# lhaippp/DMHomo

Hardware: AMD Instinct MI355X
Metric: sampled images/sec (128x128, s_step=32) (higher is better)
Workload: dtype f32; 1 GPU; DGM CFG-Unet dim=64 128x128 bs=25/GPU s_step=32 cond_scale=3 (BASELINE configs[1]); global_batch=25, cfg_mode=streams, hip_graph=True, weights=seeded random init

## Files before the change

dmhomo_amd/_lib.py:

```python
import contextlib
import ctypes as C
import gc
import os

import torch

_HERE = os.path.dirname(os.path.abspath(__file__))
LIB_PATH = os.environ.get('DMH_LIB_PATH') or os.path.join(_HERE, 'libdmhomo_hip.so')

c_f32p = C.c_void_p
c_i64 = C.c_int64
c_int = C.c_int
c_float = C.c_float


ABI_VERSION = 500


class DmhConv(C.Structure):
    _fields_ = [('struct_size', C.c_uint64)] + \
               [(n, C.c_void_p) for n in ('src0', 'src1', 'wpack', 'bias', 'in_coef', 'res', 'res_coef', 'out',
                                          'stats')] + \
               [(n, C.c_int32) for n in ('B', 'Hin', 'Win', 'C0', 'C1', 'Cout', 'KH', 'KW', 'stride', 'upsample2')] + \
               [('in_bound', C.c_void_p), ('in_bound_n', C.c_int32), ('fin_n', C.c_int32), ('fin_w', C.c_void_p),
                ('fin_b', C.c_void_p), ('fin_out', C.c_void_p), ('pix_stats', C.c_void_p), ('pix_eps', C.c_float),
                ('rows', C.c_void_p)]


class DmhPackJob(C.Structure):
    _fields_ = [('src', C.c_void_p), ('ws', C.c_void_p), ('wpack', C.c_void_p), ('Cout', C.c_int32), ('C0', C.c_int32),
                ('C1', C.c_int32), ('KH', C.c_int32), ('transposed', C.c_int32)]


class DmhStep(C.Structure):
    _fields_ = [('objective', C.c_int32), ('clip', C.c_int32), ('mode', C.c_int32), ('cond_scale', C.c_float),
                ('sqrt_recip_ac', C.c_float), ('sqrt_recipm1_ac', C.c_float), ('sqrt_ac', C.c_float),
                ('sqrt_1m_ac', C.c_float), ('c0', C.c_float), ('c1', C.c_float), ('c2', C.c_float)]


SIGNATURES = {
    'dmh_last_error': (C.c_char_p, []),
    'dmh_version': (c_int, []),
    'dmh_ws_standardize': (c_int, [c_f32p, c_f32p, c_int, c_int, c_float, C.c_void_p]),
    'dmh_conv_pack_floats': (c_i64, [c_int, c_int, c_int, c_int, c_int]),
    'dmh_pack_conv_weight': (c_int, [c_f32p, c_f32p, c_int, c_int, c_int, c_int, c_int, C.c_void_p]),
    'dmh_pack_conv_weights_multi': (c_int, [C.c_void_p, c_int, c_float, C.c_void_p]),
    'dmh_conv_up2_pack_floats': (c_i64, [c_int, c_int]),
    'dmh_pack_conv_weight_up2': (c_int, [c_f32p, c_f32p, c_int, c_int, C.c_void_p]),
    'dmh_conv_tiles': (c_int, [c_int, c_int, c_int, c_int]),
# ... 226 lines not shown
```

dmhomo_amd/csrc/common.h:

```cpp
#pragma once
#include <initializer_list>
#include <hip/hip_runtime.h>
#include <stdint.h>
#include <stdio.h>

#include "../../include/dmhomo_hip.h"

void dmh_set_error(const char* fmt, ...);

#define DMH_REQUIRE(cond, ...)   \
  do {                           \
    if (!(cond)) {               \
      dmh_set_error(__VA_ARGS__); \
      return DMH_EINVAL;         \
    }                            \
  } while (0)

#define DMH_CHECK_LAUNCH(name)                                        \
  do {                                                                \
    hipError_t e_ = hipGetLastError();                                \
    if (e_ != hipSuccess) {                                           \
      dmh_set_error("%s: launch failed: %s", name, hipGetErrorString(e_)); \
      return DMH_ELAUNCH;                                             \
    }                                                                 \
// ... 3 lines not shown
  do {                                                                                                            \
    static bool raised_ = false;                                                                                  \
    if (!raised_) {                                                                                               \
      hipError_t e_ = hipFuncSetAttribute(reinterpret_cast<const void*>(kern),                                    \
                                          hipFuncAttributeMaxDynamicSharedMemorySize, (int)(bytes));              \
      DMH_REQUIRE(e_ == hipSuccess, "%s: cannot raise the LDS limit to %d bytes: %s", name, (int)(bytes),         \
                  hipGetErrorString(e_));                                                                         \
      raised_ = true;                                                                                             \
    }                                                                                                             \
  } while (0)

static inline bool dmh_dims_ok(std::initializer_list<long long> dims, long long lo = 1, long long hi = 1 << 20) {
  for (long long d : dims)
    if (d < lo || d > hi) return false;
  return true;
}

static inline int cdiv(int a, int b) { return (a + b - 1) / b; }
static inline int64_t cdiv64(int64_t a, int64_t b) { return (a + b - 1) / b; }

__device__ __forceinline__ float silu_f(float x) { return x / (1.0f + expf(-x)); }

__device__ __forceinline__ float silu_fast(float x) { return x * __builtin_amdgcn_rcpf(1.0f + __expf(-x)); }

__device__ __forceinline__ float4 ld4(const float* p) { return *reinterpret_cast<const float4*>(p); }
__device__ __forceinline__ void st4(float* p, float4 v) { *reinterpret_cast<float4*>(p) = v; }

template <int CTRL>
__device__ __forceinline__ unsigned dmh_dpp(unsigned v) {
  return (unsigned)__builtin_amdgcn_update_dpp(0, (int)v, CTRL, 0xf, 0xf, false);
}
__device__ __forceinline__ unsigned dmh_xor16(unsigned v, unsigned* other) {
  const auto r = __builtin_amdgcn_permlane16_swap(v, v, false, false);
  *other = r[1];
  return r[0];
}
__device__ __forceinline__ unsigned dmh_xor32(unsigned v, unsigned* other) {
  const auto r = __builtin_amdgcn_permlane32_swap(v, v, false, false);
  *other = r[1];
  return r[0];
}
__device__ __forceinline__ float row16_sum(float v) {
  v += __uint_as_float(dmh_dpp<0xB1>(__float_as_uint(v)));
  v += __uint_as_float(dmh_dpp<0x4E>(__float_as_uint(v)));
  v += __uint_as_float(dmh_dpp<0x141>(__float_as_uint(v)));
  v += __uint_as_float(dmh_dpp<0x140>(__float_as_uint(v)));
// ... 76 lines not shown
```

dmhomo_amd/csrc/conv.hip:

```cpp
#include <stdlib.h>

#include "common.h"

#include "conv_args.h"
#include "weight_image.h"

template <int KH, int KW, int S, int UPS, int KC, int TH, int TW>
struct ConvCfg {
  static constexpr int BM = TH * TW;
  static constexpr int MB = BM / 128;
  static constexpr int IN_H = (TH - 1) * S + KH;
  static constexpr int IN_W = (TW - 1) * S + KW;
  static constexpr int IN_PIX = IN_H * IN_W;
  static constexpr int KCP = KC + 4;
  static constexpr int C4 = KC / 4;
  static constexpr int NLOAD = (IN_PIX * C4 + 255) / 256;
  static constexpr int WL = 64 * C4 / 256;
  static constexpr int PAD = (S == 1) ? (KH / 2) : (KH == 4 ? 1 : 0);
  static constexpr int IN_FLOATS = IN_PIX * KCP;
  static constexpr int W_FLOATS = 64 * KCP;
  static constexpr int EPI_BYTES = 4 * 32 * 68 * 4;
  static constexpr int MAIN_BYTES = (IN_FLOATS + 2 * W_FLOATS) * 4;
  static constexpr int LDS_BYTES = MAIN_BYTES > EPI_BYTES ? MAIN_BYTES : EPI_BYTES;
};
// ... 327 lines not shown
              "dmh_conv2d: input channels must be a multiple of 4 (got %d, %d)", d->C0, d->C1);
  DMH_REQUIRE(!(d->in_coef && d->src1), "dmh_conv2d: the GroupNorm prologue applies to a single source");
  DMH_REQUIRE(!(d->res_coef && !d->res), "dmh_conv2d: res_coef without res");
  DMH_REQUIRE(d->Cout % 4 == 0, "dmh_conv2d: Cout must be a multiple of 4 (got %d)", d->Cout);
  DMH_REQUIRE(!d->in_bound || (d->in_coef && d->in_bound_n > 0 && d->in_bound_n <= 64),
              "dmh_conv2d: in_bound needs in_coef and 1..64 bounds per sample (got %d)", d->in_bound_n);
  hipStream_t st = (hipStream_t)stream;
  const int Hout = conv_out_dim(d->Hin, d->KH, d->stride, d->upsample2);
  const int Wout = conv_out_dim(d->Win, d->KW, d->stride, d->upsample2);
  const int key = d->KH * 100 + d->stride * 10 + d->upsample2;
  DMH_REQUIRE(d->KH == d->KW, "dmh_conv2d: non-square kernel");
  if (d->fin_w) {
    DMH_REQUIRE(d->fin_out && d->fin_n > 0 && d->fin_n <= 8, "dmh_conv2d: fin_w needs fin_out and 1 <= fin_n <= 8 (got %d)",
                d->fin_n);
    DMH_REQUIRE(d->KH == 1 && d->stride == 1 && d->Cout <= 64 && use_f16x3(1, 1),
                "dmh_conv2d: the fused final projection rides on the 1x1 fp16-piece kernel with Cout <= 64 (got %dx%d, Cout %d)",
                d->KH, d->KW, d->Cout);
  } else {
    DMH_REQUIRE(d->out, "dmh_conv2d: null pointer");
  }
  DMH_REQUIRE(!d->pix_stats || (d->KH == 1 && d->stride == 1 && d->Cout == 64 && use_f16x3(1, 1)),
              "dmh_conv2d: pix_stats rides on the 1x1 fp16-piece kernel with Cout == 64 (got %dx%d, Cout %d)", d->KH, d->KW,
              d->Cout);
  switch (key) {
    case 110:
      if (use_f16x3(1, 1)) return dmh_f16x3_launch(d, Hout, Wout, st);
      return launch_conv<1, 1, 1, 0, 32, 16, 16>(d, Hout, Wout, st);
    case 310:
      switch (conv3_variant()) {
        case 6: return dmh_wino_launch(d, Hout, Wout, st);
        case 9: return dmh_f16x3_launch(d, Hout, Wout, st);
        default: return launch_conv<3, 3, 1, 0, 32, 16, 16, 2>(d, Hout, Wout, st);
      }
    case 311:
      switch (conv3_variant()) {
        case 6: return dmh_wino_launch(d, Hout, Wout, st);
        case 9: return dmh_f16x3_launch(d, Hout, Wout, st);
        default: return launch_conv<3, 3, 1, 1, 32, 16, 16, 2>(d, Hout, Wout, st);
      }
    case 312:
      DMH_REQUIRE(use_f16x3(3, 1) && !d->src1 && d->Cout % 64 == 0 && !d->stats,
                  "dmh_conv2d: the sub-pixel upsampling conv needs the fp16-piece kernels, one source, Cout %% 64 == 0, no stats");
      return dmh_f16x3_launch_up2(d, Hout, Wout, st);
    case 710:
      if (use_f16x3(7, 1)) return dmh_f16x3_launch(d, Hout, Wout, st);
      return launch_conv<7, 7, 1, 0, 16, 16, 16>(d, Hout, Wout, st);
// ... 15 lines not shown
```

dmhomo_amd/csrc/conv_args.h:

```cpp
#pragma once
#include "common.h"

typedef float floatx16 __attribute__((ext_vector_type(16)));

struct ConvArgs {
  const float* src0;
  const float* src1;
  const float* wpack;
  const float* bias;
  const float* in_coef;
  const float* res;
  const float* res_coef;
  float* out;
  float* stats;
  const float* oscale;
  const float* in_bound;
  int in_bound_n;
  int fin_n;
  const float* fin_w;
  const float* fin_b;
  float* fin_out;
  float* pix_stats;
  float pix_eps;
  int B, Hin, Win, C0, C1, Cout, Hout, Wout;
  int nch0, nch1, tilesX, tilesY;
  int ablate;
  int xcd;
  const int32_t* rows;
};


static inline ConvArgs fill_conv_args(const DmhConv* d, int Hout, int Wout, int KC, int TH, int TW) {
  ConvArgs a;
  a.src0 = d->src0;
  a.src1 = d->src1;
  a.wpack = d->wpack;
  a.bias = d->bias;
  a.in_coef = d->in_coef;
  a.res = d->res;
  a.res_coef = d->res_coef;
  a.out = d->out;
  a.stats = d->stats;
  a.oscale = nullptr;
  a.in_bound = d->in_coef ? d->in_bound : nullptr;
  a.in_bound_n = d->in_bound_n;
  a.fin_n = d->fin_w ? d->fin_n : 0;
  a.fin_w = d->fin_w;
  a.fin_b = d->fin_b;
  a.fin_out = d->fin_out;
  a.pix_stats = d->pix_stats;
  a.pix_eps = d->pix_eps;
  a.B = d->B;
  a.Hin = d->Hin;
  a.Win = d->Win;
  a.C0 = d->C0;
  a.C1 = d->src1 ? d->C1 : 0;
  a.Cout = d->Cout;
  a.Hout = Hout;
  a.Wout = Wout;
  a.nch0 = cdiv(a.C0, KC);
  a.nch1 = cdiv(a.C1, KC);
  a.tilesX = cdiv(Wout, TW);
  a.tilesY = cdiv(Hout, TH);
  a.ablate = 0;
  a.xcd = 1;
  a.rows = d->rows;
  return a;
}


int64_t dmh_wino_pack_floats(int Cout, int C0, int C1);
int dmh_wino_pack(const float* w, float* wpack, int Cout, int C0, int C1, hipStream_t st);
int dmh_wino_launch(const DmhConv* d, int Hout, int Wout, hipStream_t st);


int64_t dmh_f16x3_pack_floats(int Cout, int C0, int C1, int KH, int KW);
int dmh_f16x3_pack(const float* w, float* wpack, int Cout, int C0, int C1, int KH, int KW, hipStream_t st);
int dmh_f16x3_launch(const DmhConv* d, int Hout, int Wout, hipStream_t st);
int dmh_f16x3_pack_multi(const DmhPackJob* jobs, int njobs, float eps, hipStream_t st);
int64_t dmh_f16x3_up2_pack_floats(int Cout, int C0);
int dmh_f16x3_up2_pack(const float* w, float* wpack, int Cout, int C0, hipStream_t st);
int dmh_f16x3_launch_up2(const DmhConv* d, int Hout, int Wout, hipStream_t st);


struct EpilogueRows {
  static constexpr int EP = 68;
  int b, n0, chn, c4, rsub;
  bool cok;
  float4 bias, ra, rb, s1, s2, osc;
// ... 223 lines not shown
```

dmhomo_amd/csrc/conv_f16x3.hip:

```cpp
#include <stdlib.h>

#include "common.h"

#include "conv_args.h"
#include "weight_image.h"

typedef _Float16 half8 __attribute__((ext_vector_type(8)));
typedef _Float16 half4 __attribute__((ext_vector_type(4)));
typedef float float4v __attribute__((ext_vector_type(4)));

namespace {

constexpr int KC = 32;
constexpr int PITCH = 160;
constexpr int STEP_U4 = 4 * 64;

template <int KH, int KW, int S, int UPS, int TH, int TW, int WM, int WN>
struct F16Cfg {
  static_assert(WM * WN == 4, "four waves per workgroup");
  static constexpr bool SUB = UPS == 3;
  static_assert(SUB || TH * TW == WM * 64, "64 pixels per wave");
  static_assert(!SUB || (KH == 2 && KW == 2 && S == 1 && TH == 4 && TW == 16 && WM == 4 && WN == 1), "sub-pixel geometry");
  static constexpr int IN_H = SUB ? TH + 2 : (TH - 1) * S + KH;
  static constexpr int IN_W = SUB ? TW + 2 : (TW - 1) * S + KW;
  static constexpr int IN_PIX = IN_H * IN_W;
  static constexpr int QS = UPS == 4 ? 2 : 3, NQ = 1 << QS;
  static constexpr int NLOAD = (IN_PIX * NQ + 255) / 256;
  static constexpr int PAD = UPS == 2 ? 0 : ((S == 1) ? (KH / 2) : (KH == 4 ? 1 : 0));
  static constexpr int ROWP = IN_W * PITCH;
  static constexpr int IN_BYTES = IN_H * ROWP;
  static constexpr int EPI_BYTES = 4 * 32 * EpilogueRows::EP * 4;
  static constexpr int TILE_BYTES = IN_BYTES > EPI_BYTES ? IN_BYTES : EPI_BYTES;
  static constexpr int LDS_BYTES = TILE_BYTES + 16;
};

__device__ __forceinline__ unsigned absbits(float x) { return __float_as_uint(x) & 0x7fffffffu; }

__device__ __forceinline__ int64_t f16x3_frag_floats_dev(int Cout, int C0, int C1, int T) {
  return (int64_t)((Cout + 63) / 64) * ((C0 + KC - 1) / KC + (C1 + KC - 1) / KC) * T * 2 * STEP_U4 * 4;
}

}

template <int KH, int KW, int S, int UPS, int TH, int TW, int WM, int WN>
__global__ __launch_bounds__(256, 2) void conv_f16x3_kernel(ConvArgs p) {
  using Cfg = F16Cfg<KH, KW, S, UPS, TH, TW, WM, WN>;
  constexpr bool PK = UPS == 4;
  constexpr int IN_W = Cfg::IN_W, IN_PIX = Cfg::IN_PIX, NLOAD = Cfg::NLOAD, NTAPS = PK ? (KH * KW + 1) / 2 : KH * KW,
                ROWP = Cfg::ROWP;

  extern __shared__ __attribute__((aligned(16))) float lds[];
  unsigned char* in_tile = reinterpret_cast<unsigned char*>(lds);
  unsigned* mxslot = reinterpret_cast<unsigned*>(in_tile + Cfg::TILE_BYTES);

  const int tid = threadIdx.x;
  const int lane = tid & 63;
  const int wave = tid >> 6;
  const int wave_u = __builtin_amdgcn_readfirstlane(wave);
  const int kg = lane >> 4;
  const int l15 = lane & 15;
  const int wm = wave / WN, wn = wave % WN;

  int t = blockIdx.x, by = blockIdx.y, nb = gridDim.x;
  if (p.rows) {
    nb = p.tilesX * p.tilesY * p.rows[0];
    const int lin = t + by * (int)gridDim.x;
    if (lin >= nb * (int)gridDim.y) return;
    t = lin % nb;
    by = lin / nb;
  }
// ... 51 lines not shown
#pragma unroll
    for (int nb = 0; nb < 4; ++nb) acc[mb][nb] = float4v{0.f, 0.f, 0.f, 0.f};

  const int nchunks = p.nch0 + p.nch1;
  const int nsteps = nchunks * NTAPS * 2;
  const uint4* wbase = reinterpret_cast<const uint4*>(p.wpack) + (size_t)__builtin_amdgcn_readfirstlane(nt) * nsteps * STEP_U4;

  constexpr bool ROWREUSE = KH == 3 && KW == 3 && S == 1 && UPS != 3 && UPS != 2;
  constexpr int NSTEP = NTAPS * 2;
  constexpr int NB = (NSTEP % 3 == 0 && WN != 1) ? 3 : 2;
  uint4 bq[NB][4];
  auto tap_of = [](int pos) constexpr { return ROWREUSE ? (pos % 3) * 3 + pos / 3 : pos; };
  auto load_b = [&](int buf, int ch_, int st_) {
    if (st_ >= NSTEP) {
      st_ -= NSTEP;
      ch_ += 1;
    }
    if (ch_ >= nchunks) ch_ = nchunks - 1;
    const uint4* src = wbase + ((size_t)(ch_ * NTAPS + tap_of(st_ >> 1)) * 2 + (st_ & 1)) * STEP_U4;
#pragma unroll
    for (int i = 0; i < 4; ++i) bq[buf][i] = src[i * 64 + lane];
  };
#pragma unroll
  for (int i = 0; i < NB - 1; ++i) load_b(i, 0, i);

  constexpr int QS = Cfg::QS, NQ = Cfg::NQ;
  const int c4 = tid & (NQ - 1);
  float4 v[NLOAD];
  constexpr bool PACKPW = KH == 3 && KW == 3 && S == 1 && UPS == 0 && WN == 1;
  int poff[NLOAD], wroff[PACKPW ? 1 : NLOAD];
  const int y0c = min(max(iy0, 0), Hlim - 1), x0c = min(max(ix0, 0), Wlim - 1);
  const int pbase = PACKPW ? (b * p.Hin + y0c) * p.Win + x0c : 0;
  unsigned inside = 0;
#pragma unroll
  for (int i = 0; i < NLOAD; ++i) {
    const int pix = (tid + i * 256) >> QS;
    const int pixc = pix < IN_PIX ? pix : IN_PIX - 1;
    const int wro = (pixc / IN_W) * ROWP + (pixc % IN_W) * PITCH + c4 * 8;
    if (!PACKPW) wroff[i] = wro;
    const int yy = iy0 + pixc / IN_W, xx = ix0 + pixc % IN_W;
    const bool ok = pix < IN_PIX && yy >= 0 && yy < Hlim && xx >= 0 && xx < Wlim;
    const int yc = min(max(yy, 0), Hlim - 1), xc = min(max(xx, 0), Wlim - 1);
    const int sy = UPS == 1 ? (yc >> 1) : yc, sx = UPS == 1 ? (xc >> 1) : xc;
    poff[i] = UPS == 2 ? ((yc << 16) | xc) : (b * p.Hin + sy) * p.Win + sx;
    if (PACKPW) poff[i] = (int)((unsigned)wro | ((unsigned)((yc - y0c) * p.Win + (xc - x0c)) << 16));
    inside |= (ok ? 1u : 0u) << i;
  }
  unsigned inside_ch = inside;
  const float* ld_src = p.src0;
  int ld_C = p.C0, ld_c = 0, ld_py = 0, ld_px = 0;
  auto issue_prep = [&](int ch) {
    const bool s1 = ch >= p.nch0;
    ld_src = s1 ? p.src1 : p.src0;
    ld_C = s1 ? p.C1 : p.C0;
    if (UPS == 2) {
      const int nchc = p.C0 / KC, par = ch / nchc;
      ld_py = par >> 1;
      ld_px = par & 1;
      ld_c = (ch - par * nchc) * KC + c4 * 4;
      inside_ch = 0u;
    } else {
      const int c = (s1 ? ch - p.nch0 : ch) * KC + c4 * 4;
      ld_c = c < ld_C ? c : 0;
    }
  };
  auto issue_one = [&](int i) {
    const float* a;
    if (UPS == 2) {
      const int ry = 2 * (poff[i] >> 16) - 1 + ld_py, rx = 2 * (poff[i] & 0xffff) - 1 + ld_px;
      const bool ok = ((inside >> i) & 1u) && ry >= 0 && ry < p.Hin && rx >= 0 && rx < p.Win;
      const int yc = min(max(ry, 0), p.Hin - 1), xc = min(max(rx, 0), p.Win - 1);
      a = ld_src + ((size_t)(b * p.Hin + yc) * p.Win + xc) * ld_C + ld_c;
      inside_ch |= (ok ? 1u : 0u) << i;
    } else {
      if (PACKPW) a = ld_src + (size_t)pbase * ld_C + (int)(((unsigned)poff[i] >> 16) * (unsigned)ld_C + (unsigned)ld_c);
      else a = ld_src + (size_t)poff[i] * ld_C + ld_c;
    }
#ifdef DMH_STAMPS
    a = (p.ablate & 32) ? ld_src + ld_c : a;
#endif
    v[i] = ld4(a);
  };
  issue_prep(0);
#pragma unroll
  for (int i = 0; i < NLOAD; ++i) issue_one(i);
  __syncthreads();
#ifdef DMH_STAMPS
  if (p.ablate & 128) {
    const float* gs = p.src0 + (size_t)b * p.Hin * p.Win * p.C0;
    double q1 = 0.0, q2 = 0.0;
#pragma unroll
    for (int j = 0; j < 4; ++j) {
      const float2 t2 = *reinterpret_cast<const float2*>(gs + (size_t)(((tid & 31) + 32 * j) * 8 + (tid >> 5)) * 2);
      q1 += (double)t2.x;
      q2 += (double)t2.y;
    }
    for (int off = 16; off; off >>= 1) {
      q1 += __shfl_xor(q1, off);
      q2 += __shfl_xor(q2, off);
    }
    const double nn = (double)p.Hin * p.Win * (p.C0 / 8);
    const double mean = q1 / nn;
    double var = q2 / nn - mean * mean;
    var = var < 0.0 ? 0.0 : var;
// ... 35 lines not shown
  }
  for (int ch = 0; ch < nchunks; ++ch) {
    const bool s1c = ch >= p.nch0;
    const bool pro = (p.in_coef != nullptr) && !s1c;
    float4 ca = make_float4(1.f, 1.f, 1.f, 1.f), cb = make_float4(0.f, 0.f, 0.f, 0.f);
    if (pro) {
      const int cq = ch * KC + c4 * 4;
      const int ccq = cq < p.C0 ? cq : 0;
      ca = ld4(p.in_coef + (size_t)(b * 2 + 0) * p.C0 + ccq);
      cb = ld4(p.in_coef + (size_t)(b * 2 + 1) * p.C0 + ccq);
    }
    const bool cvalid = UPS == 2 || (s1c ? ch - p.nch0 : ch) * KC + c4 * 4 < (s1c ? p.C1 : p.C0);
    const unsigned msk = cvalid ? inside_ch : 0u;
    if (pro) {
#pragma unroll
      for (int i = 0; i < NLOAD; ++i) {
        if ((i + 1) * 256 > IN_PIX * NQ && ((wave_u * 64 + i * 256) >> QS) >= IN_PIX) continue;
        v[i].x = silu_fast(fmaf(ca.x, v[i].x, cb.x));
        v[i].y = silu_fast(fmaf(ca.y, v[i].y, cb.y));
        v[i].z = silu_fast(fmaf(ca.z, v[i].z, cb.z));
        v[i].w = silu_fast(fmaf(ca.w, v[i].w, cb.w));
      }
    }
    if (!stat) {
      float mxf = 0.f;
#pragma unroll
      for (int i = 0; i < NLOAD; ++i) {
        if (pro && (i + 1) * 256 > IN_PIX * NQ && ((wave_u * 64 + i * 256) >> QS) >= IN_PIX) continue;
        mxf = fmaxf(fmaxf(mxf, fmaxf(fabsf(v[i].x), fabsf(v[i].y))), fmaxf(fabsf(v[i].z), fabsf(v[i].w)));
      }
      unsigned mx = __float_as_uint(mxf);
      mx = wave_max_u32(mx);
      if (lane == 0) atomicMax(&mxslot[ch & 1], mx);
    }
    STAMP(0)
    __syncthreads();
    STAMP(1)
    const int e_old = e_run;
    int e_ch = e_fix;
    if (!stat) {
      const unsigned bmx = mxslot[ch & 1];
      if (tid == 0) mxslot[(ch + 1) & 1] = 0u;
      e_ch = min(max((int)(__builtin_amdgcn_readfirstlane(bmx) >> 23), 16), 254);
    }
    e_run = max(e_run, e_ch);
    const float sc = __uint_as_float((unsigned)(268 - e_run) << 23);
    if (e_run != e_old && ch > 0) {
      const int fe = 127 + e_old - e_run;
      const float f = fe > 0 ? __uint_as_float((unsigned)fe << 23) : 0.f;
#pragma unroll
      for (int mb = 0; mb < 4; ++mb)
#pragma unroll
        for (int nb = 0; nb < 4; ++nb) acc[mb][nb] *= f;
    }
    const bool more = ch + 1 < nchunks;
    if (more) issue_prep(ch + 1);
#ifdef DMH_STAMPS
    if (p.ablate & 1) {
#pragma unroll
      for (int i = 0; i < NLOAD; ++i)
        if (more) issue_one(i);
    } else
#endif
#pragma unroll
    for (int i = 0; i < NLOAD; ++i) {
      if ((i + 1) * 256 <= IN_PIX * NQ || ((tid + i * 256) >> QS) < IN_PIX) {
        const float si = ((msk >> i) & 1u) ? sc : 0.f;
        uint2 h1, h2;
        dmh_split2(v[i].x, v[i].y, si, h1.x, h2.x);
        dmh_split2(v[i].z, v[i].w, si, h1.y, h2.y);
        int slot = PACKPW ? poff[i] : wroff[i];
        if (PACKPW) asm volatile("v_and_b32 %0, 0xffff, %0" : "+v"(slot));
        unsigned char* dst = in_tile + slot;
        *reinterpret_cast<uint2*>(dst) = h1;
        *reinterpret_cast<uint2*>(dst + 64) = h2;
      }
      if (more) issue_one(i);
    }
    STAMP(2)
    __syncthreads();
    STAMP(3)
    __builtin_amdgcn_sched_barrier(0);

    half8 a[4][2];
    half8 ar[ROWREUSE ? 5 : 1][2];
    auto read_a = [&](int tap) {
      const unsigned char* at = in_tile + (tap / KW) * ROWP + (tap % KW) * PITCH;
      if constexpr (PK) {
        const int t0 = 2 * tap, t1 = 2 * tap + 1 < KH * KW ? 2 * tap + 1 : 2 * tap;
        const int o0 = (t0 / KW) * ROWP + (t0 % KW) * PITCH, o1 = (t1 / KW) * ROWP + (t1 % KW) * PITCH;
        at = in_tile + ((kg >> 1) ? o1 : o0);
      }
#pragma unroll
      for (int mb = 0; mb < 4; ++mb)
#pragma unroll
        for (int pl = 0; pl < 2; ++pl) a[mb][pl] = *reinterpret_cast<const half8*>(at + arow[mb] + pl * 64);
    };
    auto read_rows = [&](int kx, int r0, int r1) {
      const unsigned char* at = in_tile + kx * PITCH;
#pragma unroll
      for (int r = r0; r < r1; ++r)
#pragma unroll
        for (int pl = 0; pl < 2; ++pl)
          ar[ROWREUSE ? r % 5 : 0][pl] = *reinterpret_cast<const half8*>(at + arow[0] + r * ROWP + pl * 64);
    };
#ifdef DMH_STAMPS
    if (!(p.ablate & 2))
#endif
    {
#pragma unroll
      for (int st = 0; st < NSTEP; ++st) {
#ifdef DMH_STAMPS
        if (!(p.ablate & 8))
#endif
        load_b((st + NB - 1) % NB, ch, st + NB - 1);
        __builtin_amdgcn_sched_barrier(0);
        const int pos = st >> 1;
#ifdef DMH_STAMPS
        if (!(p.ablate & 16) || st == 0)
#endif
        {
          if (ROWREUSE) {
            if ((st & 1) == 0) read_rows(pos / 3, pos % 3 == 0 ? 0 : 3 + pos % 3, 4 + pos % 3);
          } else if ((st & 1) == 0) {
            read_a(pos);
          }
        }
        auto afrag = [&](int mb, int pl) -> half8 {
          if constexpr (ROWREUSE) return ar[(mb + pos % 3) % 5][pl];
          else return a[mb][pl];
        };
#define DMH_A(mb, pl) afrag(mb, pl)
#pragma unroll
        for (int mb = 0; mb < 4; ++mb)
#pragma unroll
          for (int nb = 0; nb < 2; ++nb) {
            float4v& c = acc[mb][(st & 1) * 2 + nb];
            const half8 g1 = __builtin_bit_cast(half8, bq[st % NB][nb * 2]), g2 = __builtin_bit_cast(half8, bq[st % NB][nb * 2 + 1]);
            const half8 h1 = DMH_A(mb, 0), h2 = DMH_A(mb, 1);
            asm("v_mfma_f32_16x16x32_f16 %0, %1, %4, %0\n\t"
                "v_mfma_f32_16x16x32_f16 %0, %2, %3, %0\n\t"
                "v_mfma_f32_16x16x32_f16 %0, %1, %3, %0"
                : "+v"(c) : "v"(g1), "v"(g2), "v"(h1), "v"(h2));
          }
#undef DMH_A
      }
    }
#pragma unroll
    for (int mb = 0; mb < 4; mb += 2)
      asm volatile("s_nop 15" : "+v"(acc[mb][0]), "+v"(acc[mb][1]), "+v"(acc[mb][2]), "+v"(acc[mb][3]), "+v"(acc[mb + 1][0]),
                   "+v"(acc[mb + 1][1]), "+v"(acc[mb + 1][2]), "+v"(acc[mb + 1][3]));
    __builtin_amdgcn_sched_barrier(0);
    STAMP(4)
  }

#ifdef DMH_STAMPS
  if (!(p.ablate & 4))
#endif
  {
    constexpr int EP = EpilogueRows::EP;
    const float inv_s = __uint_as_float((unsigned)(e_run - 14) << 23);
    float* wl = lds + wave * (32 * EP);
    EpilogueRows er(p, b, n0);
    if (UPS == 3 && p.oscale) er.osc = ld4(p.oscale + nt * 64 + er.c4 * 4);
    er.osc.x *= inv_s;
    er.osc.y *= inv_s;
    er.osc.z *= inv_s;
    er.osc.w *= inv_s;
    __syncthreads();
#pragma unroll
    for (int hb = 0; hb < 2; ++hb) {
#pragma unroll
      for (int m2 = 0; m2 < 2; ++m2)
#pragma unroll
        for (int nb = 0; nb < 4; ++nb)
// ... 236 lines not shown
  return DMH_OK;
}

int dmh_f16x3_launch(const DmhConv* d, int Hout, int Wout, hipStream_t st) {
  const bool wide = d->Cout % 128 == 0;
  if (d->KH == 4) {
    return wide ? launch_f16x3<2, 2, 1, 2, 8, 16, 2, 2>(d, Hout, Wout, st)
                : launch_f16x3<2, 2, 1, 2, 16, 16, 4, 1>(d, Hout, Wout, st);
  }
  if (d->KH == 7) {
    if (f16x3_pk(d->C0, d->src1 ? d->C1 : 0, 7)) return launch_f16x3<7, 7, 1, 4, 16, 16, 4, 1>(d, Hout, Wout, st);
    return launch_f16x3<7, 7, 1, 0, 16, 16, 4, 1>(d, Hout, Wout, st);
  }
  if (d->KH == 1) {
    return wide ? launch_f16x3<1, 1, 1, 0, 8, 16, 2, 2>(d, Hout, Wout, st)
                : launch_f16x3<1, 1, 1, 0, 16, 16, 4, 1>(d, Hout, Wout, st);
  }
  if (d->upsample2) {
    return wide ? launch_f16x3<3, 3, 1, 1, 8, 16, 2, 2>(d, Hout, Wout, st)
                : launch_f16x3<3, 3, 1, 1, 16, 16, 4, 1>(d, Hout, Wout, st);
  }
  if (wide) return launch_f16x3<3, 3, 1, 0, 8, 16, 2, 2>(d, Hout, Wout, st);
  DMH_REQUIRE(17 * (int64_t)d->Win + 17 < 65536, "dmh_conv2d: 3x3 with Cout %% 128 != 0 supports Win <= 3853 (got %d)", d->Win);
  return launch_f16x3<3, 3, 1, 0, 16, 16, 4, 1>(d, Hout, Wout, st);
}
```

dmhomo_amd/csrc/norm.hip:

```cpp
#include "common.h"

__global__ __launch_bounds__(256) void gn_finalize_kernel(const float* __restrict__ stats, int tiles,
                                                          const float* __restrict__ gamma,
                                                          const float* __restrict__ beta, const float* __restrict__ ss,
                                                          int64_t ss_stride, float* __restrict__ coef, int C, int groups,
                                                          int hw, float eps, float* __restrict__ mr,
                                                          float* __restrict__ bound, const int32_t* __restrict__ rows) {
  __shared__ double red[2][4];
  __shared__ float bred[4];
  const int jb = blockIdx.x / groups, g = blockIdx.x % groups;
  if (jb >= dmh_rows_n(rows, gridDim.x / groups)) return;
  const int b = dmh_rows_phys(rows, jb);
  const int bg = b * groups + g;
  const int cg = C / groups;
  const int lane = threadIdx.x;
  double s1 = 0.0, s2 = 0.0;
  const int total = tiles * cg;
  for (int i = lane; i < total; i += 256) {
    const int tile = i / cg, cc = i % cg;
    const float2 st = *reinterpret_cast<const float2*>(stats + ((size_t)(b * tiles + tile) * C + g * cg + cc) * 2);
    s1 += (double)st.x;
    s2 += (double)st.y;
  }
  for (int off = 32; off; off >>= 1) {
// ... 45 lines not shown
__global__ __launch_bounds__(256) void gn_silu_residual_kernel(const float* __restrict__ y,
                                                               const float* __restrict__ coef,
                                                               const float* __restrict__ res, float* __restrict__ out,
                                                               int64_t per_sample4, int C, int64_t total4_all,
                                                               float* __restrict__ pstats, float eps,
                                                               const int32_t* __restrict__ rows) {
  const int C4 = C >> 2;
  const int lane = threadIdx.x & 63;
  const int64_t total4 = rows ? per_sample4 * rows[0] : total4_all;
  for (int64_t i0 = (int64_t)blockIdx.x * 256 + threadIdx.x; i0 - lane < total4; i0 += (int64_t)gridDim.x * 256) {
    const bool ok = i0 < total4;
    if (LPP == 0 && !ok) break;
    const int64_t il = ok ? i0 : total4 - 1;
    const int jb = (int)(il / per_sample4);
    const int b = dmh_rows_phys(rows, jb);
    const int64_t i = il + (int64_t)(b - jb) * per_sample4;
    const int c = (int)(i % C4) * 4;
    const float4 a = ld4(coef + (size_t)(b * 2 + 0) * C + c);
    const float4 bb = ld4(coef + (size_t)(b * 2 + 1) * C + c);
    const float4 v = ld4(y + i * 4);
    float4 r = make_float4(0.f, 0.f, 0.f, 0.f);
    if (res) r = ld4(res + i * 4);
    float4 o;
    o.x = silu_fast(fmaf(a.x, v.x, bb.x)) + r.x;
    o.y = silu_fast(fmaf(a.y, v.y, bb.y)) + r.y;
    o.z = silu_fast(fmaf(a.z, v.z, bb.z)) + r.z;
    o.w = silu_fast(fmaf(a.w, v.w, bb.w)) + r.w;
    if (ok) st4(out + i * 4, o);
    if (LPP > 0) {
      float s = 0.f;
      s += (o.x + o.y) + (o.z + o.w);
      s = lanes_sum<(LPP > 0 ? LPP : 1)>(s);
      const float mean = s / (float)C;
      float qsum = 0.f;
      const float dx = o.x - mean, dy = o.y - mean, dz = o.z - mean, dw = o.w - mean;
      qsum += (dx * dx + dy * dy) + (dz * dz + dw * dw);
      qsum = lanes_sum<(LPP > 0 ? LPP : 1)>(qsum);
      if (ok && (threadIdx.x % (LPP > 0 ? LPP : 1)) == 0) {
        const int64_t pix = i / C4;
        pstats[pix * 2 + 0] = mean;
        pstats[pix * 2 + 1] = 1.0f / sqrtf(qsum / (float)C + eps);
      }
    }
  }
}

template <int LPP, int NV>
__global__ __launch_bounds__(256) void chan_layernorm_kernel(const float* __restrict__ x, const float* __restrict__ g,
                                                             const float* __restrict__ res, float* __restrict__ out,
                                                             int64_t npix_all, int C, float eps,
// ... 216 lines not shown
```

dmhomo_amd/engine.py:

```python
import torch

from . import ops
from .layout import ATTN_SCALE, HIDDEN, sinusoidal_freq, unet_layout

FUSED_FINAL = True


class _Res:
    __slots__ = ('conv1', 'g1', 'b1', 'conv2', 'g2', 'b2', 'res', 'ss_off', 'cout')


class _Attn:
    __slots__ = ('linear', 'ln_g', 'qkv', 'pla', 'plo', 'out', 'out_g')


class UnetEngine:
    def __init__(self, module, groups=8):
        self.module = module
        self.groups = groups
        self._sig = None
        self._rows = None
        self._pert_lo = None

    def _signature(self):
        return (getattr(self.module, '_dmh_epoch', 0),) + tuple((p.data_ptr(), p._version) for p in self.module.parameters())

    def ensure_prepared(self):
        sig = self._signature()
# ... 65 lines not shown

        self.blocks = []
        for n in L.nodes:
            k = n.keys
            if n.kind == 'res':
                b = res(n)
            elif n.kind in ('linattn', 'attn'):
                b = attn(n)
            elif n.kind == 'unshuffle':
                w22 = f32(k['w']).reshape(n.cout, n.c0, 2, 2).contiguous()
                b = ops.PackedConv(w22, f32(k['b']), n.c0, 0, stride=2, batch=pb)
            else:
                b = conv(k['w'], k['b'], n.c0, stride=2 if n.kind == 'down4' else 1, ups=1 if n.kind == 'up3' else 0)
            self.blocks.append((n, b))
        pb.run()
        nxt = [b for _, b in self.blocks[1:]] + [None]
        self._pixel_stats = [isinstance(a, _Attn) and a.pla is not None for a in nxt]
        self.final_w = f32('final_conv.weight').reshape(L.out_dim, -1).contiguous()
        self.final_b = f32('final_conv.bias')
        res_nodes = [n for n in L.nodes if n.kind == 'res']
        self.mlp_wt = torch.cat([f32(n.keys['mlp_w']).t() for n in res_nodes], dim=1).contiguous()
        self.mlp_b = torch.cat([f32(n.keys['mlp_b']) for n in res_nodes]).contiguous()

    def _res(self, r, x0, x1, ss_all, pixel_stats=False, pre=None, final=None, keep_out=True, fin_out=None):
        B, H, W, _ = x0.shape
        hw = H * W
        rows = self._rows
        y1, st1 = pre if pre is not None else ops.conv2d(r.conv1, x0, x1, want_stats=True, rows=rows)
        ss = ss_all[:, r.ss_off:r.ss_off + 2 * r.cout]
        coef1, bound1 = ops.gn_finalize(st1, r.g1, r.b1, hw, self.groups, ss, want_bound=True, rows=rows)
        y2, st2 = ops.conv2d(r.conv2, y1, in_coef=coef1, want_stats=True, in_bound=bound1, rows=rows)
        coef2 = ops.gn_finalize(st2, r.g2, r.b2, hw, self.groups, rows=rows)
        if final is not None:
            return ops.conv2d(r.res, x0, x1, res=y2, res_coef=coef2, final=final, keep_out=keep_out, fin_out=fin_out, rows=rows)
        if r.res is not None:
            if pixel_stats and r.cout == 64 and r.res.k == 1 and ops.f16x3_default():
                return ops.conv2d(r.res, x0, x1, res=y2, res_coef=coef2, pixel_stats=True, rows=rows)
            x = ops.conv2d(r.res, x0, x1, res=y2, res_coef=coef2, rows=rows)
            return (x, None) if pixel_stats else x
        assert x1 is None
        if pixel_stats:
            if r.cout in ops.PIXEL_STATS_FUSABLE:
                return ops.gn_silu_residual(y2, coef2, x0, pixel_stats=True, rows=rows)
            return ops.gn_silu_residual(y2, coef2, x0, rows=rows), None
        return ops.gn_silu_residual(y2, coef2, x0, rows=rows)

    def _attn(self, a, x, stats=None):
        rows = self._rows
        if a.plo is not None:
            return ops.linear_attention_fused(x, a.ln_g, a.pla, ATTN_SCALE, out=a.plo, stats=stats, rows=rows)
        if a.pla is not None:
            o = ops.linear_attention_fused(x, a.ln_g, a.pla, ATTN_SCALE, stats=stats, rows=rows)
            y = ops.conv2d(a.out, o, rows=rows)
            return ops.chan_layernorm(y, a.out_g, res=x, rows=rows)
        xn = ops.chan_layernorm(x, a.ln_g, rows=rows)
        qkv = ops.conv2d(a.qkv, xn, rows=rows)
        if a.linear:
            o = ops.linear_attention_core(qkv, ATTN_SCALE, rows=rows)
            y = ops.conv2d(a.out, o, rows=rows)
            return ops.chan_layernorm(y, a.out_g, res=x, rows=rows)
        o = ops.attention_core(qkv, ATTN_SCALE, rows=rows, pert_lo=self._pert_lo)
        return ops.conv2d(a.out, o, res=x, rows=rows)

    def embed(self, time, class_rows, reps):
        B = time.shape[0]
        td = self.t_w2.shape[1]
        cond = torch.empty((reps * B, self.emb_dim), device=time.device, dtype=torch.float32)
        se = ops.fourier_embed(time, self.fourier_w) if self.fourier_w is not None else ops.sinusoidal_embed(time, self.freq)
# ... 31 lines not shown
    def first_conv(self, x0):
        self.ensure_prepared()
        return ops.conv2d(self.blocks[0][1].conv1, x0, None, want_stats=True)

    def trunk(self, x0, cond, taps=None, first=None, out=None, ss_all=None, rows=None, pert_lo=None):
        self.ensure_prepared()
        self._rows, self._pert_lo = rows, pert_lo
        try:
            return self._trunk(x0, cond, taps, first, out, ss_all)
        finally:
            self._rows = self._pert_lo = None

    def _trunk(self, x0, cond, taps, first, out, ss_all):
        rows = self._rows

        def tap(name, v):
            if taps is not None:
                taps[name] = v
            return v
        if ss_all is None:
            ss_all = ops.linear(cond, self.mlp_wt, self.mlp_b, act_in='silu')
        x = tap('init_conv', x0)
        hs, pst, last = [x], None, len(self.blocks) - 1
        for i, (n, b) in enumerate(self.blocks):
            x1 = hs.pop() if n.c1 else None
            if n.kind == 'res':
                if i == last and FUSED_FINAL and b.res is not None and b.res.k == 1 and b.cout <= 64 \
                        and self.final_w.shape[0] <= 8 and ops.f16x3_default():
                    x, y = self._res(b, x, x1, ss_all, final=(self.final_w, self.final_b), keep_out=taps is not None,
                                     fin_out=out)
                    tap(n.name, x)
                    return y
                if self._pixel_stats[i]:
                    x, pst = self._res(b, x, x1, ss_all, pixel_stats=True)
                else:
                    x = self._res(b, x, x1, ss_all, pre=first if i == 0 else None)
            elif n.kind in ('linattn', 'attn'):
                x, pst = self._attn(b, x, pst), None
            else:
                x = ops.conv2d(b, x, rows=rows)
            tap(n.name, x)
            if n.push:
                hs.append(x)
        y = ops.final_conv_nchw(x, self.final_w, self.final_b)
        if out is not None:
            out.copy_(y)
            return out
        return y
```

dmhomo_amd/ops.py:

```python
import ctypes as C
import math

import os

import torch

from . import _lib
from ._lib import call, ptr, lib

F32 = torch.float32


def _empty(shape, like, dtype=F32):
    return torch.empty(shape, device=like.device, dtype=dtype)


def ws_standardize(w, eps=1e-5, out=None):
    w = w.detach().contiguous()
    out = torch.empty_like(w) if out is None else out
    cout = w.shape[0]
    call('dmh_ws_standardize', ptr(w), ptr(out), cout, w.numel() // cout, float(eps))
    return out


# ... 70 lines not shown
def conv_out_hw(pc, h, w):
    if pc.upsample2:
        return h * 2, w * 2
    if pc.stride == 2:
        return h // 2, w // 2
    return h, w


CONV_LOG = None


def rows_from_keep(keep, extra=0):
    B = keep.shape[0]
    rows = torch.empty((1 + B + extra,), device=keep.device, dtype=torch.int32)
    call('dmh_rows_from_keep', ptr(keep, torch.uint8), B, int(extra), ptr(rows, torch.int32))
    return rows


def _rows(rows):
    return ptr(rows, torch.int32)


def conv2d(pc, src0, src1=None, in_coef=None, res=None, res_coef=None, want_stats=False, in_bound=None, final=None,
           keep_out=True, pixel_stats=False, eps=1e-5, fin_out=None, rows=None):
    B, H, W, c0 = src0.shape
    assert c0 == pc.c0 and (pc.c1 == 0) == (src1 is None), (src0.shape, pc.c0, pc.c1)
    if src1 is not None:
        assert src1.shape == (B, H, W, pc.c1), (src1.shape, pc.c1)
    ho, wo = conv_out_hw(pc, H, W)
    assert keep_out or final is not None
    out = _empty((B, ho, wo, pc.cout), src0) if keep_out else None
    fin_w = fin_b = None
    if final is not None:
        fin_w, fin_b = final
        assert fin_w.shape[1] == pc.cout and fin_w.is_contiguous() and not want_stats, (fin_w.shape, pc.cout)
        if fin_out is None:
            fin_out = _empty((B, fin_w.shape[0], ho, wo), src0)
        assert fin_out.shape == (B, fin_w.shape[0], ho, wo) and fin_out.is_contiguous() and fin_out.dtype == F32
    else:
        assert fin_out is None
    pst = None
    if pixel_stats:
        assert final is None and not want_stats and pc.cout == 64 and pc.k == 1, (pc.cout, pc.k)
        pst = _empty((B, ho * wo, 2), src0)
    stats = None
    if want_stats:
        tiles = lib().dmh_conv_tiles(ho, wo, pc.k, pc.stride)
        stats = _empty((B, tiles, pc.cout, 2), src0)
    if res is not None:
        assert res.shape == (B, ho, wo, pc.cout), (res.shape, (B, ho, wo, pc.cout))
    d = _lib.DmhConv(C.sizeof(_lib.DmhConv), ptr(src0), ptr(src1), ptr(pc.wpack), ptr(pc.bias), ptr(in_coef), ptr(res), ptr(res_coef),
                     ptr(out), ptr(stats), B, H, W, pc.c0, pc.c1, pc.cout, pc.k, pc.k, pc.stride, pc.upsample2,
                     ptr(in_bound), 0 if in_bound is None else in_bound.shape[1],
                     0 if fin_w is None else fin_w.shape[0], ptr(fin_w), ptr(fin_b), ptr(fin_out), ptr(pst), float(eps), _rows(rows))
    if CONV_LOG is not None:
        e0, e1 = torch.cuda.Event(enable_timing=True), torch.cuda.Event(enable_timing=True)
        e0.record()
        call('dmh_conv2d', C.byref(d))
        e1.record()
        CONV_LOG.append((e0, e1, pc.k, pc.stride, B, ho, wo, pc.c0 + pc.c1, pc.cout, pc.upsample2, in_coef is not None))
    else:
        call('dmh_conv2d', C.byref(d))
    if final is not None:
        return out, fin_out
    if pixel_stats:
        return out, pst
    return (out, stats) if want_stats else out


def _ss_arg(ss, B, Cc):
    if ss is None:
        return None, 0
    assert ss.stride(1) == 1 and ss.shape[0] == B and ss.shape[1] == 2 * Cc
    return C.c_void_p(ss.data_ptr()), ss.stride(0)


def gn_finalize(stats, gamma, beta, hw, groups, ss=None, eps=1e-5, want_bound=False, rows=None):
    B, tiles, Cc, _ = stats.shape
    coef = _empty((B, 2, Cc), stats)
    ss_ptr, ss_stride = _ss_arg(ss, B, Cc)
    if want_bound:
        bound = _empty((B, groups), stats)
        call('dmh_gn_finalize_bound', ptr(stats), tiles, ptr(gamma), ptr(beta), ss_ptr, ss_stride, ptr(coef), ptr(bound),
             B, Cc, groups, hw, float(eps), _rows(rows))
        return coef, bound
    call('dmh_gn_finalize', ptr(stats), tiles, ptr(gamma), ptr(beta), ss_ptr, ss_stride, ptr(coef), B, Cc, groups,
         hw, float(eps), _rows(rows))
    return coef

# ... 1143 lines not shown
```

include/dmhomo_hip.h:

```cpp
#ifndef DMHOMO_HIP_H
#define DMHOMO_HIP_H

#include <stdint.h>

#ifdef __cplusplus
extern "C" {
#endif

#define DMH_OK 0
#define DMH_EINVAL (-1)
#define DMH_ELAUNCH (-2)

const char* dmh_last_error(void);
#define DMH_ABI_VERSION 500
int dmh_version(void);


int dmh_ws_standardize(const float* w, float* w_out, int Cout, int K, float eps, void* stream);

int64_t dmh_conv_pack_floats(int Cout, int C0, int C1, int KH, int KW);

int dmh_pack_conv_weight(const float* w_oihw, float* wpack, int Cout, int C0, int C1, int KH, int KW,
                         void* stream);
typedef struct DmhPackJob {
// ... 14 lines not shown
  uint64_t struct_size;
  const float* src0;
  const float* src1;
  const float* wpack;
  const float* bias;
  const float* in_coef;
  const float* res;
  const float* res_coef;
  float* out;
  float* stats;
  int32_t B, Hin, Win, C0, C1, Cout;
  int32_t KH, KW;
  int32_t stride;
  int32_t upsample2;
  const float* in_bound;
  int32_t in_bound_n;
  int32_t fin_n;
  const float* fin_w;
  const float* fin_b;
  float* fin_out;
  float* pix_stats;
  float pix_eps;
  const int32_t* rows;
} DmhConv;

int dmh_conv_tiles(int Hout, int Wout, int KH, int stride);
int dmh_conv2d(const DmhConv* d, void* stream);


int dmh_gn_finalize(const float* stats, int tiles, const float* gamma, const float* beta, const float* ss,
                    int64_t ss_stride, float* coef, int B, int C, int groups, int hw, float eps, const int32_t* rows,
                    void* stream);

int dmh_gn_finalize_bound(const float* stats, int tiles, const float* gamma, const float* beta, const float* ss,
                          int64_t ss_stride, float* coef, float* bound, int B, int C, int groups, int hw, float eps,
                          const int32_t* rows, void* stream);

int dmh_gn_silu_residual(const float* y, const float* coef, const float* res, float* out, int B, int HW, int C,
                         const int32_t* rows, void* stream);

int dmh_gn_silu_residual_stats(const float* y, const float* coef, const float* res, float* out, float* pstats, int B,
                               int HW, int C, float eps, const int32_t* rows, void* stream);

int dmh_chan_layernorm(const float* x, const float* g, const float* res, float* out, int64_t npix, int C,
                       float eps, const int32_t* rows, int64_t pix_per_row, void* stream);

// ... 241 lines not shown
```

Measured before the change: 88.26 images/s.

## Fuse residual block GroupNorm-SiLU-residual finish into next block's 3x3 conv prologue

Defers the GroupNorm+SiLU+residual finish of a residual block (Cout<=64, no shortcut conv) and performs it inside the next block's first 3x3 conv load stage. The conv loads the pre-norm activation and the residual, applies the affine, SiLU and add, stores the finished tile interior to ff_out for the skip/residual path, and uses the result as conv input. This removes a separate elementwise kernel launch and one read of the activation, at the cost of a new kernel variant. That variant drops the weight prefetch overlap (B loads start only after staging), issues the next input loads after the MMA loop, and does extra global stores in the prologue.

Result: no change. 88.75 images/s, median of 6 (+0.6%).

```diff
diff --git a/dmhomo_amd/_lib.py b/dmhomo_amd/_lib.py
--- a/dmhomo_amd/_lib.py
+++ b/dmhomo_amd/_lib.py
@@ -24,7 +24,7 @@
                [(n, C.c_int32) for n in ('B', 'Hin', 'Win', 'C0', 'C1', 'Cout', 'KH', 'KW', 'stride', 'upsample2')] + \
                [('in_bound', C.c_void_p), ('in_bound_n', C.c_int32), ('fin_n', C.c_int32), ('fin_w', C.c_void_p),
                 ('fin_b', C.c_void_p), ('fin_out', C.c_void_p), ('pix_stats', C.c_void_p), ('pix_eps', C.c_float),
-                ('rows', C.c_void_p)]
+                ('rows', C.c_void_p), ('ff_y', C.c_void_p), ('ff_coef', C.c_void_p), ('ff_out', C.c_void_p)]
 
 
 class DmhPackJob(C.Structure):
diff --git a/dmhomo_amd/csrc/common.h b/dmhomo_amd/csrc/common.h
--- a/dmhomo_amd/csrc/common.h
+++ b/dmhomo_amd/csrc/common.h
@@ -49,6 +49,11 @@
 __device__ __forceinline__ float silu_f(float x) { return x / (1.0f + expf(-x)); }
 
 __device__ __forceinline__ float silu_fast(float x) { return x * __builtin_amdgcn_rcpf(1.0f + __expf(-x)); }
+
+__device__ __forceinline__ float gn_silu_res(float a, float y, float b, float r) {
+  const float z = fmaf(a, y, b);
+  return fmaf(z, __builtin_amdgcn_rcpf(1.0f + __expf(-z)), r);
+}
 
 __device__ __forceinline__ float4 ld4(const float* p) { return *reinterpret_cast<const float4*>(p); }
 __device__ __forceinline__ void st4(float* p, float4 v) { *reinterpret_cast<float4*>(p) = v; }
diff --git a/dmhomo_amd/csrc/conv.hip b/dmhomo_amd/csrc/conv.hip
--- a/dmhomo_amd/csrc/conv.hip
+++ b/dmhomo_amd/csrc/conv.hip
@@ -373,6 +373,18 @@
   DMH_REQUIRE(!d->pix_stats || (d->KH == 1 && d->stride == 1 && d->Cout == 64 && use_f16x3(1, 1)),
               "dmh_conv2d: pix_stats rides on the 1x1 fp16-piece kernel with Cout == 64 (got %dx%d, Cout %d)", d->KH, d->KW,
               d->Cout);
+  if (d->ff_y || d->ff_coef || d->ff_out) {
+    DMH_REQUIRE(d->ff_y && d->ff_coef && d->ff_out, "dmh_conv2d: the fused finish needs ff_y, ff_coef and ff_out together");
+    DMH_REQUIRE(key == 310 && d->Cout <= 64 && conv3_variant() == 9,
+                "dmh_conv2d: the fused finish rides on the plain stride-1 3x3 fp16-piece kernel with Cout <= 64 (got %dx%d, "
+                "stride %d, upsample2 %d, Cout %d)", d->KH, d->KW, d->stride, d->upsample2, d->Cout);
+    DMH_REQUIRE(!d->src1, "dmh_conv2d: the fused finish takes a single source");
+    DMH_REQUIRE(!d->in_coef, "dmh_conv2d: the fused finish takes no GroupNorm prologue");
+    const size_t nin = (size_t)d->B * d->Hin * d->Win * d->C0, nout = (size_t)d->B * Hout * Wout * d->Cout;
+    auto overlaps = [&](const float* q, size_t n) { return q && q < d->ff_out + nin && d->ff_out < q + n; };
+    DMH_REQUIRE(!overlaps(d->src0, nin) && !overlaps(d->ff_y, nin) && !overlaps(d->out, nout) && !overlaps(d->res, nout),
+                "dmh_conv2d: ff_out overlaps src0, ff_y, res or out");
+  }
   switch (key) {
     case 110:
       if (use_f16x3(1, 1)) return dmh_f16x3_launch(d, Hout, Wout, st);
diff --git a/dmhomo_amd/csrc/conv_args.h b/dmhomo_amd/csrc/conv_args.h
--- a/dmhomo_amd/csrc/conv_args.h
+++ b/dmhomo_amd/csrc/conv_args.h
@@ -27,6 +27,9 @@
   int ablate;
   int xcd;
   const int32_t* rows;
+  const float* ff_y;
+  const float* ff_coef;
+  float* ff_out;
 };
 
 
@@ -65,6 +68,9 @@
   a.ablate = 0;
   a.xcd = 1;
   a.rows = d->rows;
+  a.ff_y = d->ff_y;
+  a.ff_coef = d->ff_coef;
+  a.ff_out = d->ff_out;
   return a;
 }
 
diff --git a/dmhomo_amd/csrc/conv_f16x3.hip b/dmhomo_amd/csrc/conv_f16x3.hip
--- a/dmhomo_amd/csrc/conv_f16x3.hip
+++ b/dmhomo_amd/csrc/conv_f16x3.hip
@@ -46,6 +46,8 @@
 __global__ __launch_bounds__(256, 2) void conv_f16x3_kernel(ConvArgs p) {
   using Cfg = F16Cfg<KH, KW, S, UPS, TH, TW, WM, WN>;
   constexpr bool PK = UPS == 4;
+  constexpr bool FF = UPS == 5;
+  static_assert(!FF || (KH == 3 && KW == 3 && S == 1 && TH == 16 && WN == 1), "the fused finish rides on the plain 16x16x64 3x3");
   constexpr int IN_W = Cfg::IN_W, IN_PIX = Cfg::IN_PIX, NLOAD = Cfg::NLOAD, NTAPS = PK ? (KH * KW + 1) / 2 : KH * KW,
                 ROWP = Cfg::ROWP;
 
@@ -143,16 +145,18 @@
     for (int i = 0; i < 4; ++i) bq[buf][i] = src[i * 64 + lane];
   };
 #pragma unroll
-  for (int i = 0; i < NB - 1; ++i) load_b(i, 0, i);
+  for (int i = 0; i < (FF ? 0 : NB - 1); ++i) load_b(i, 0, i);
 
   constexpr int QS = Cfg::QS, NQ = Cfg::NQ;
   const int c4 = tid & (NQ - 1);
   float4 v[NLOAD];
-  constexpr bool PACKPW = KH == 3 && KW == 3 && S == 1 && UPS == 0 && WN == 1;
+  constexpr bool PACKPW = KH == 3 && KW == 3 && S == 1 && (UPS == 0 || FF) && WN == 1;
   int poff[NLOAD], wroff[PACKPW ? 1 : NLOAD];
   const int y0c = min(max(iy0, 0), Hlim - 1), x0c = min(max(ix0, 0), Wlim - 1);
   const int pbase = PACKPW ? (b * p.Hin + y0c) * p.Win + x0c : 0;
   unsigned inside = 0;
+  float4 rx[FF ? NLOAD : 1];
+  unsigned interior = 0;
 #pragma unroll
   for (int i = 0; i < NLOAD; ++i) {
     const int pix = (tid + i * 256) >> QS;
@@ -166,6 +170,10 @@
     poff[i] = UPS == 2 ? ((yc << 16) | xc) : (b * p.Hin + sy) * p.Win + sx;
     if (PACKPW) poff[i] = (int)((unsigned)wro | ((unsigned)((yc - y0c) * p.Win + (xc - x0c)) << 16));
     inside |= (ok ? 1u : 0u) << i;
+    if (FF) {
+      const int py = pixc / IN_W, px = pixc % IN_W;
+      interior |= ((ok && py >= 1 && py <= TH && px >= 1 && px <= TW) ? 1u : 0u) << i;
+    }
   }
   unsigned inside_ch = inside;
   const float* ld_src = p.src0;
@@ -201,6 +209,13 @@
     a = (p.ablate & 32) ? ld_src + ld_c : a;
 #endif
     v[i] = ld4(a);
+    if constexpr (FF) {
+      rx[i] = v[i];
+      v[i] = ld4(p.ff_y + (size_t)pbase * ld_C + (int)(((unsigned)poff[i] >> 16) * (unsigned)ld_C + (unsigned)ld_c));
+    }
+  };
+  auto ff_dst = [&](int i) -> float* {
+    return p.ff_out + (size_t)pbase * ld_C + (int)(((unsigned)poff[i] >> 16) * (unsigned)ld_C + (unsigned)ld_c);
   };
   issue_prep(0);
 #pragma unroll
@@ -282,11 +297,28 @@
         v[i].w = silu_fast(fmaf(ca.w, v[i].w, cb.w));
       }
     }
+    if constexpr (FF) {
+      const int cq = ch * KC + c4 * 4;
+      const int ccq = cq < p.C0 ? cq : 0;
+      const float4 fa = ld4(p.ff_coef + (size_t)(b * 2 + 0) * p.C0 + ccq);
+      const float4 fb = ld4(p.ff_coef + (size_t)(b * 2 + 1) * p.C0 + ccq);
+      const unsigned stm = cvalid ? interior : 0u;
+#pragma unroll
+      for (int i = 0; i < NLOAD; ++i) {
+        if ((i + 1) * 256 > IN_PIX * NQ && ((wave_u * 64 + i * 256) >> QS) >= IN_PIX) continue;
+        v[i].x = gn_silu_res(fa.x, v[i].x, fb.x, rx[i].x);
+        v[i].y = gn_silu_res(fa.y, v[i].y, fb.y, rx[i].y);
+        v[i].z = gn_silu_res(fa.z, v[i].z, fb.z, rx[i].z);
+        v[i].w = gn_silu_res(fa.w, v[i].w, fb.w, rx[i].w);
+        if ((stm >> i) & 1u) st4(ff_dst(i), v[i]);
+        __builtin_amdgcn_sched_barrier(0);
+      }
+    }
     if (!stat) {
       float mxf = 0.f;
 #pragma unroll
       for (int i = 0; i < NLOAD; ++i) {
-        if (pro && (i + 1) * 256 > IN_PIX * NQ && ((wave_u * 64 + i * 256) >> QS) >= IN_PIX) continue;
+        if ((pro || FF) && (i + 1) * 256 > IN_PIX * NQ && ((wave_u * 64 + i * 256) >> QS) >= IN_PIX) continue;
         mxf = fmaxf(fmaxf(mxf, fmaxf(fabsf(v[i].x), fabsf(v[i].y))), fmaxf(fabsf(v[i].z), fabsf(v[i].w)));
       }
       unsigned mx = __float_as_uint(mxf);
@@ -319,7 +351,7 @@
     if (p.ablate & 1) {
 #pragma unroll
       for (int i = 0; i < NLOAD; ++i)
-        if (more) issue_one(i);
+        if (!FF && more) issue_one(i);
     } else
 #endif
 #pragma unroll
@@ -335,8 +367,9 @@
         *reinterpret_cast<uint2*>(dst) = h1;
         *reinterpret_cast<uint2*>(dst + 64) = h2;
       }
-      if (more) issue_one(i);
-    }
+      if (!FF && more) issue_one(i);
+    }
+    if constexpr (FF) load_b(0, ch, 0);
     STAMP(2)
     __syncthreads();
     STAMP(3)
@@ -373,6 +406,7 @@
 #ifdef DMH_STAMPS
         if (!(p.ablate & 8))
 #endif
+        if (!FF || st + NB - 1 < NSTEP)
         load_b((st + NB - 1) % NB, ch, st + NB - 1);
         __builtin_amdgcn_sched_barrier(0);
         const int pos = st >> 1;
@@ -411,6 +445,12 @@
       asm volatile("s_nop 15" : "+v"(acc[mb][0]), "+v"(acc[mb][1]), "+v"(acc[mb][2]), "+v"(acc[mb][3]), "+v"(acc[mb + 1][0]),
                    "+v"(acc[mb + 1][1]), "+v"(acc[mb + 1][2]), "+v"(acc[mb + 1][3]));
     __builtin_amdgcn_sched_barrier(0);
+    if constexpr (FF) {
+      if (more) {
+#pragma unroll
+        for (int i = 0; i < NLOAD; ++i) issue_one(i);
+      }
+    }
     STAMP(4)
   }
 
@@ -693,5 +733,6 @@
   }
   if (wide) return launch_f16x3<3, 3, 1, 0, 8, 16, 2, 2>(d, Hout, Wout, st);
   DMH_REQUIRE(17 * (int64_t)d->Win + 17 < 65536, "dmh_conv2d: 3x3 with Cout %% 128 != 0 supports Win <= 3853 (got %d)", d->Win);
+  if (d->ff_out) return launch_f16x3<3, 3, 1, 5, 16, 16, 4, 1>(d, Hout, Wout, st);
   return launch_f16x3<3, 3, 1, 0, 16, 16, 4, 1>(d, Hout, Wout, st);
 }
diff --git a/dmhomo_amd/csrc/norm.hip b/dmhomo_amd/csrc/norm.hip
--- a/dmhomo_amd/csrc/norm.hip
+++ b/dmhomo_amd/csrc/norm.hip
@@ -91,10 +91,10 @@
     float4 r = make_float4(0.f, 0.f, 0.f, 0.f);
     if (res) r = ld4(res + i * 4);
     float4 o;
-    o.x = silu_fast(fmaf(a.x, v.x, bb.x)) + r.x;
-    o.y = silu_fast(fmaf(a.y, v.y, bb.y)) + r.y;
-    o.z = silu_fast(fmaf(a.z, v.z, bb.z)) + r.z;
-    o.w = silu_fast(fmaf(a.w, v.w, bb.w)) + r.w;
+    o.x = gn_silu_res(a.x, v.x, bb.x, r.x);
+    o.y = gn_silu_res(a.y, v.y, bb.y, r.y);
+    o.z = gn_silu_res(a.z, v.z, bb.z, r.z);
+    o.w = gn_silu_res(a.w, v.w, bb.w, r.w);
     if (ok) st4(out + i * 4, o);
     if (LPP > 0) {
       float s = 0.f;
diff --git a/dmhomo_amd/engine.py b/dmhomo_amd/engine.py
--- a/dmhomo_amd/engine.py
+++ b/dmhomo_amd/engine.py
@@ -4,6 +4,7 @@
 from .layout import ATTN_SCALE, HIDDEN, sinusoidal_freq, unet_layout
 
 FUSED_FINAL = True
+FUSED_FINISH = True
 
 
 class _Res:
@@ -115,7 +116,7 @@
         self.mlp_wt = torch.cat([f32(n.keys['mlp_w']).t() for n in res_nodes], dim=1).contiguous()
         self.mlp_b = torch.cat([f32(n.keys['mlp_b']) for n in res_nodes]).contiguous()
 
-    def _res(self, r, x0, x1, ss_all, pixel_stats=False, pre=None, final=None, keep_out=True, fin_out=None):
+    def _res(self, r, x0, x1, ss_all, pixel_stats=False, pre=None, final=None, keep_out=True, fin_out=None, defer=False):
         B, H, W, _ = x0.shape
         hw = H * W
         rows = self._rows
@@ -132,11 +133,22 @@
             x = ops.conv2d(r.res, x0, x1, res=y2, res_coef=coef2, rows=rows)
             return (x, None) if pixel_stats else x
         assert x1 is None
+        if defer:
+            return y2, coef2
         if pixel_stats:
             if r.cout in ops.PIXEL_STATS_FUSABLE:
                 return ops.gn_silu_residual(y2, coef2, x0, pixel_stats=True, rows=rows)
             return ops.gn_silu_residual(y2, coef2, x0, rows=rows), None
         return ops.gn_silu_residual(y2, coef2, x0, rows=rows)
+
+    def _defers_finish(self, i, taps):
+        n, b = self.blocks[i]
+        if not FUSED_FINISH or taps is not None or b.res is not None or n.c1 or b.cout > 64 or self._pixel_stats[i]:
+            return False
+        if i + 1 >= len(self.blocks) or not ops.f16x3_default():
+            return False
+        nn_ = self.blocks[i + 1][0]
+        return nn_.kind == 'res' and nn_.c1 == 0
 
     def _attn(self, a, x, stats=None):
         rows = self._rows
@@ -214,19 +226,29 @@
             ss_all = ops.linear(cond, self.mlp_wt, self.mlp_b, act_in='silu')
         x = tap('init_conv', x0)
         hs, pst, last = [x], None, len(self.blocks) - 1
+        pend = None
         for i, (n, b) in enumerate(self.blocks):
             x1 = hs.pop() if n.c1 else None
+            pre = first if i == 0 else None
+            if pend is not None:
+                y1, st1, x = ops.conv2d(b.conv1, x, want_stats=True, rows=rows, finish=pend[:2])
+                if pend[2]:
+                    hs.append(x)
+                pre, pend = (y1, st1), None
+            if n.kind == 'res' and self._defers_finish(i, taps):
+                pend = self._res(b, x, x1, ss_all, pre=pre, defer=True) + (n.push,)
+                continue
             if n.kind == 'res':
                 if i == last and FUSED_FINAL and b.res is not None and b.res.k == 1 and b.cout <= 64 \
                         and self.final_w.shape[0] <= 8 and ops.f16x3_default():
-                    x, y = self._res(b, x, x1, ss_all, final=(self.final_w, self.final_b), keep_out=taps is not None,
+                    x, y = self._res(b, x, x1, ss_all, pre=pre, final=(self.final_w, self.final_b), keep_out=taps is not None,
                                      fin_out=out)
                     tap(n.name, x)
                     return y
                 if self._pixel_stats[i]:
-                    x, pst = self._res(b, x, x1, ss_all, pixel_stats=True)
+                    x, pst = self._res(b, x, x1, ss_all, pixel_stats=True, pre=pre)
                 else:
-                    x = self._res(b, x, x1, ss_all, pre=first if i == 0 else None)
+                    x = self._res(b, x, x1, ss_all, pre=pre)
             elif n.kind in ('linattn', 'attn'):
                 x, pst = self._attn(b, x, pst), None
             else:
diff --git a/dmhomo_amd/ops.py b/dmhomo_amd/ops.py
--- a/dmhomo_amd/ops.py
+++ b/dmhomo_amd/ops.py
@@ -116,7 +116,7 @@
 
 
 def conv2d(pc, src0, src1=None, in_coef=None, res=None, res_coef=None, want_stats=False, in_bound=None, final=None,
-           keep_out=True, pixel_stats=False, eps=1e-5, fin_out=None, rows=None):
+           keep_out=True, pixel_stats=False, eps=1e-5, fin_out=None, rows=None, finish=None):
     B, H, W, c0 = src0.shape
     assert c0 == pc.c0 and (pc.c1 == 0) == (src1 is None), (src0.shape, pc.c0, pc.c1)
     if src1 is not None:
@@ -143,10 +143,18 @@
         stats = _empty((B, tiles, pc.cout, 2), src0)
     if res is not None:
         assert res.shape == (B, ho, wo, pc.cout), (res.shape, (B, ho, wo, pc.cout))
+    ff_y = ff_coef = ff_out = None
+    if finish is not None:
+        ff_y, ff_coef = finish[:2]
+        assert final is None and not pixel_stats and ff_y.shape == src0.shape and ff_coef.shape == (B, 2, c0), \
+            (ff_y.shape, ff_coef.shape, src0.shape)
+        ff_out = finish[2] if len(finish) > 2 else torch.empty_like(src0)
+        assert ff_out.shape == src0.shape and ff_out.is_contiguous() and ff_out.dtype == F32
     d = _lib.DmhConv(C.sizeof(_lib.DmhConv), ptr(src0), ptr(src1), ptr(pc.wpack), ptr(pc.bias), ptr(in_coef), ptr(res), ptr(res_coef),
                      ptr(out), ptr(stats), B, H, W, pc.c0, pc.c1, pc.cout, pc.k, pc.k, pc.stride, pc.upsample2,
                      ptr(in_bound), 0 if in_bound is None else in_bound.shape[1],
-                     0 if fin_w is None else fin_w.shape[0], ptr(fin_w), ptr(fin_b), ptr(fin_out), ptr(pst), float(eps), _rows(rows))
+                     0 if fin_w is None else fin_w.shape[0], ptr(fin_w), ptr(fin_b), ptr(fin_out), ptr(pst), float(eps), _rows(rows),
+                     ptr(ff_y), ptr(ff_coef), ptr(ff_out))
     if CONV_LOG is not None:
         e0, e1 = torch.cuda.Event(enable_timing=True), torch.cuda.Event(enable_timing=True)
         e0.record()
@@ -159,6 +167,8 @@
         return out, fin_out
     if pixel_stats:
         return out, pst
+    if finish is not None:
+        return (out, stats, ff_out) if want_stats else (out, ff_out)
     return (out, stats) if want_stats else out
 
 
diff --git a/include/dmhomo_hip.h b/include/dmhomo_hip.h
--- a/include/dmhomo_hip.h
+++ b/include/dmhomo_hip.h
@@ -60,6 +60,9 @@
   float* pix_stats;
   float pix_eps;
   const int32_t* rows;
+  const float* ff_y;
+  const float* ff_coef;
+  float* ff_out;
 } DmhConv;
 
 int dmh_conv_tiles(int Hout, int Wout, int KH, int stride);
```
